# IST-DASLab/qutlass

Measured on AMD Instinct MI355X. Metric: TFLOP/s & %FP4-MFMA-peak, MXFP4 GEMM 4096x4096x4096, 1 MI355X, higher is better.
Workload: dtype fp4 (e2m1 x e2m1, e8m0 block scales, fp32 accumulate, bf16 out); 1 GPU; matmul_mxf4_bf16_tn 4096x4096x4096, gs=32 e8m0 scales (BASELINE.json configs[1]); parallelism=single GPU, clock_ramp=8000 untimed steps (~250 ms) before the 5 warmup steps

## Files before the change

qutlass_amd/csrc/capi.hip:

```cpp
#include <hip/hip_runtime.h>

#include <algorithm>
#include <atomic>
#include <chrono>
#include <cstdarg>
#include <cstdio>
#include <cstring>

#include "../../include/qutlass_amd.h"
#include "gemm_mx.hip.h"
#include "gemm_mx_deepp.hip.h"
#if QAMD_BENCH
#include "lab/gemm_mx_duo.hip.h"
#include "lab/gemm_mx_deepp_lab.hip.h"
#endif
#include "gemm_mx_skinny.hip.h"
#include "gemm_mx_ks.hip.h"
#include "gemm_mx_os.hip.h"
#include "gemm_mx_fusedq.hip.h"
#include "gemm_nvf4.hip.h"
#include "gemm_nvf4_pk.hip.h"
#include "gemm_nvf4_os.hip.h"
#include "quantize.hip.h"
#include "moe_route.hip.h"
#include "to_blocked.hip.h"
#include "transpose_u8.hip.h"
#include "quartet_bwd.hip.h"
#if QAMD_BENCH
#include "lab/quartet_bwd_lab.hip.h"
#endif

using namespace qamd;

#ifndef QAMD_TU
#define QAMD_TU 0
#endif
#define QAMD_DEF(n) (QAMD_TU == 0 || QAMD_TU == (n))
#ifndef QAMD_BENCH
#define QAMD_BENCH 0
#endif

namespace qamd_host {

#if QAMD_DEF(1)
thread_local char g_err[512] = "";
#if QAMD_BENCH
std::atomic<int> g_hw_fp4_cvt{1};
std::atomic<int> g_gemm_variant{0};
std::atomic<int> g_nvf4_variant{0};
std::atomic<int> g_splitk_wg{0};
std::atomic<int> g_splitk_min_kt{32};
std::atomic<int> g_transpose_nc{0};
std::atomic<int> g_pp_shift{2};
std::atomic<int> g_pp_flags{1};
std::atomic<int> g_quant_wg_per_cu{0};
std::atomic<int> g_deepp_grid{0};
std::atomic<int> g_bwd_variant{0};
std::atomic<int> g_moe_sort_one_launch_max{0};
std::atomic<int> g_splitk_force{0};
std::atomic<uint32_t*> g_dbg{nullptr};
#endif

int fail(int code, const char* fmt, ...) {
  va_list ap;
  va_start(ap, fmt);
  vsnprintf(g_err, sizeof(g_err), fmt, ap);
  va_end(ap);
  return code;
}

int check_launch(const char* what) {
  hipError_t e = hipGetLastError();
  if (e != hipSuccess) return fail(QAMD_ERR_HIP, "%s: %s", what, hipGetErrorString(e));
  return QAMD_OK;
}

unsigned long long next_launch_tag() {
  static std::atomic<unsigned long long> tag{[] {
    unsigned long long x = (unsigned long long)std::chrono::steady_clock::now().time_since_epoch().count() ^ ((unsigned long long)(uintptr_t)&g_err << 17);
    x ^= x >> 31; x *= 0x9e3779b97f4a7c15ull; x ^= x >> 29;
    return x | 1ull;
  }()};
  return tag.fetch_add(1, std::memory_order_relaxed) + 1;
}
#else
unsigned long long next_launch_tag();
#if QAMD_BENCH
extern std::atomic<int> g_hw_fp4_cvt, g_gemm_variant, g_nvf4_variant, g_splitk_wg, g_splitk_min_kt, g_transpose_nc, g_pp_shift, g_pp_flags, g_quant_wg_per_cu, g_splitk_force, g_deepp_grid, g_bwd_variant, g_moe_sort_one_launch_max;
extern std::atomic<uint32_t*> g_dbg;
#endif
int fail(int code, const char* fmt, ...);
int check_launch(const char* what);
#endif

#if QAMD_BENCH
inline bool opt_hw_fp4() { return g_hw_fp4_cvt.load() != 0; }
inline int opt_gemm_variant() { return g_gemm_variant.load(); }
inline int opt_nvf4_variant() { return g_nvf4_variant.load(); }
inline int opt_splitk_wg() { return g_splitk_wg.load(); }
inline int opt_splitk_min_kt() { return g_splitk_min_kt.load(); }
inline int opt_transpose_nc() { return g_transpose_nc.load(); }
inline int opt_pp_shift() { return g_pp_shift.load(); }
inline int opt_pp_flags() { return g_pp_flags.load(); }
inline int opt_quant_wg_per_cu() { return g_quant_wg_per_cu.load(); }
inline int opt_splitk_force() { return g_splitk_force.load(); }
inline int opt_deepp_grid() { return g_deepp_grid.load(); }
inline int opt_bwd_variant() { return g_bwd_variant.load(); }
inline int opt_moe_sort_one_launch_max() { return g_moe_sort_one_launch_max.load(); }
inline uint32_t* opt_dbg() { return g_dbg.load(); }
#else
constexpr bool opt_hw_fp4() { return true; }
constexpr int opt_gemm_variant() { return 0; }
constexpr int opt_nvf4_variant() { return 0; }
constexpr int opt_splitk_wg() { return 0; }
constexpr int opt_splitk_min_kt() { return 32; }
constexpr int opt_transpose_nc() { return 0; }
constexpr int opt_pp_shift() { return 2; }
constexpr int opt_pp_flags() { return 1; }
constexpr int opt_quant_wg_per_cu() { return 0; }
constexpr int opt_splitk_force() { return 0; }
constexpr int opt_deepp_grid() { return 0; }
constexpr int opt_bwd_variant() { return 0; }
constexpr int opt_moe_sort_one_launch_max() { return 0; }
constexpr uint32_t* opt_dbg() { return nullptr; }
#endif

inline int64_t cdiv(int64_t a, int64_t b) { return (a + b - 1) / b; }

#if QAMD_DEF(1)
int chip_cus() {
  static std::atomic<int> cache[64];
  int dev = 0;
  if (hipGetDevice(&dev) != hipSuccess || dev < 0 || dev >= 64) return 256;
  int v = cache[dev].load(std::memory_order_relaxed);
  if (v <= 0) {
    int n = 0;
    if (hipDeviceGetAttribute(&n, hipDeviceAttributeMultiprocessorCount, dev) != hipSuccess || n <= 0) n = 256;
// ... 834 lines not shown
  if (M * N >= (1ll << 40) || M >= (1ll << 31) || N >= (1ll << 31)) return fail(QAMD_ERR_INVALID, "%s: an output of 2^40 elements is not supported", name);
  return QAMD_OK;
}

template <int EBITS>
int gemm_mx(const char* name, const void* A, const void* B, const void* A_sf, const void* B_sf,
            const float* alpha, void* D, int64_t M, int64_t N, int64_t K, void* stream, void* ws = nullptr, int64_t ws_bytes = 0, int a_fmt = 0) {
  if (int rc = mx_check(name, EBITS, A, B, A_sf, B_sf, alpha, D, M, N, K)) return rc;
  const MxArgs x{A, B, A_sf, B_sf, alpha, D, K, N, EBITS, false};
  return for_each_range(name, M, N, K * EBITS / 8, 256, [&](int64_t r0, int64_t c0, int64_t m, int64_t n) -> int {
    const MxPlan pl = mx_plan<EBITS>(a_fmt, m, n, K, N, ws ? ws_bytes : 0, chip_cus());
    for (int i = 0; i < pl.n; ++i)
      if (int rc = mx_launch<EBITS>(name, pl.l[i], mx_params(x, r0, c0 + pl.l[i].c0, m, pl.l[i].n), ws, a_fmt, (hipStream_t)stream)) return rc;
    return QAMD_OK;
  });
}

template <class P>
int debug_plan(const char* name, int64_t M, int64_t N, int64_t rowbytes, int gran, int* out, int cap, P&& plan) {
  int cnt = 0;
  const int rc = for_each_range(name, M, N, rowbytes, gran, [&](int64_t, int64_t, int64_t m, int64_t n) {
    const MxPlan pl = plan(m, n);
    for (int i = 0; i < pl.n; ++i, ++cnt)
      if (cnt < 8 && cnt < cap) { out[3 * cnt] = pl.l[i].variant; out[3 * cnt + 1] = (int)pl.l[i].n; out[3 * cnt + 2] = pl.l[i].splits; }
    return QAMD_OK;
  });
  return rc == QAMD_OK ? cnt : -1;
}

#endif

enum QuantKind { QK_PLAIN, QK_GATED, QK_GATHER, QK_GATED_GSCALE, QK_GATHER_GSCALE };

template <int KIND, int R, bool NV, int METHOD, bool MASK, bool BLK>
int launch_quant(const QuantParams& p, hipStream_t s, int grid) {
  static_assert((KIND != QK_GATED_GSCALE && KIND != QK_GATHER_GSCALE) || (NV && METHOD == METHOD_ABSMAX && !MASK && !BLK), "per-expert global scales: NV abs-max, flat scales");
  if constexpr (KIND == QK_GATED_GSCALE) {
    hipLaunchKernelGGL((fused_silu_mul_quantize_gscale_kernel<R>), dim3(grid), dim3(256), 0, s, p);
    return check_launch("fused_silu_mul_quantize_gscale_kernel");
  } else if constexpr (KIND == QK_GATHER_GSCALE) {
    hipLaunchKernelGGL((fused_gather_quantize_gscale_kernel<R>), dim3(grid), dim3(256), 0, s, p);
    return check_launch("fused_gather_quantize_gscale_kernel");
  } else if constexpr (KIND == QK_GATED) {
    hipLaunchKernelGGL((fused_silu_mul_quantize_kernel<R, NV, METHOD, BLK>), dim3(grid), dim3(256), 0, s, p);
    return check_launch("fused_silu_mul_quantize_kernel");
  } else if constexpr (KIND == QK_GATHER) {
    hipLaunchKernelGGL((fused_gather_quantize_kernel<R, NV, METHOD>), dim3(grid), dim3(256), 0, s, p);
    return check_launch("fused_gather_quantize_kernel");
  } else {
#if QAMD_BENCH
    if (!opt_hw_fp4()) hipLaunchKernelGGL((fused_quantize_kernel<R, NV, METHOD, MASK, false, BLK>), dim3(grid), dim3(256), 0, s, p);
    else
#endif
    hipLaunchKernelGGL((fused_quantize_kernel<R, NV, METHOD, MASK, true, BLK>), dim3(grid), dim3(256), 0, s, p);
    return check_launch("fused_quantize_kernel");
  }
}

template <int KIND, bool NV, int METHOD, bool MASK, bool BLK>
int dispatch_quant(int rot, const QuantParams& p, hipStream_t s, int grid, const char* name) {
  static_assert(!MASK || (KIND == QK_PLAIN && !NV && METHOD == METHOD_QUEST), "the clip mask exists for the plain MX quest quantizer only");
  static_assert(!BLK || (KIND != QK_GATHER && KIND != QK_GATED_GSCALE && KIND != QK_GATHER_GSCALE), "the gathering and the grouped-scale quantizers write flat scales only");
  switch (rot) {
    case 16:
      if constexpr (NV) return launch_quant<KIND, 16, NV, METHOD, false, BLK>(p, s, grid);
      break;
    case 32: return launch_quant<KIND, 32, NV, METHOD, MASK, BLK>(p, s, grid);
    case 64:
      if constexpr (!MASK) return launch_quant<KIND, 64, NV, METHOD, false, BLK>(p, s, grid);
// ... 46 lines not shown
  if (which == 4) {
    if (!hw) { QAMD_BWD_GO((bwd_qt_panel_kernel<false>), 512); return check_launch("bwd_qt_panel_kernel"); }
    QAMD_BWD_GO((bwd_qt_panel_kernel<true>), 512);
    return check_launch("bwd_qt_panel_kernel");
  }
#endif
  if (which == 1) {
#if QAMD_BENCH
    if (!hw) { if (qt) QAMD_BWD_GO((bwd_quant_t_kernel<true, false>), 512); else QAMD_BWD_GO((bwd_quant_t_kernel<false, false>), 512); return check_launch("bwd_quant_t_kernel"); }
#endif
    if (qt) QAMD_BWD_GO((bwd_quant_t_kernel<true, true>), 512); else QAMD_BWD_GO((bwd_quant_t_kernel<false, true>), 512);
    return check_launch("bwd_quant_t_kernel");
  }
#if QAMD_BENCH
  if (!hw) {
    if (which == 3) { if (qt) QAMD_BWD_GO((bwd_quant_tw_kernel<true, false, 8>), 256); else QAMD_BWD_GO((bwd_quant_tw_kernel<false, false, 8>), 256); }
    else            { if (qt) QAMD_BWD_GO((bwd_quant_tw_kernel<true, false, 4>), 256); else QAMD_BWD_GO((bwd_quant_tw_kernel<false, false, 4>), 256); }
    return check_launch("bwd_quant_tw_kernel");
  }
  if (which == 9) {
    if (qt) QAMD_BWD_GO((bwd_quant_tw_kernel<true, true, 2>), 256); else QAMD_BWD_GO((bwd_quant_tw_kernel<false, true, 2>), 256);
    return check_launch("bwd_quant_tw_kernel");
  }
  if (qt && which == 3) { QAMD_BWD_GO((bwd_quant_tw_kernel<true, true, 8>), 256); return check_launch("bwd_quant_tw_kernel"); }
  if (!qt && which == 2) { QAMD_BWD_GO((bwd_quant_tw_kernel<false, true, 4>), 256); return check_launch("bwd_quant_tw_kernel"); }
#endif
  if (qt) QAMD_BWD_GO((bwd_quant_tw_kernel<true, true, 4>), 256); else QAMD_BWD_GO((bwd_quant_tw_kernel<false, true, 8>), 256);
#undef QAMD_BWD_GO
  return check_launch("bwd_quant_tw_kernel");
}
#endif

#if QAMD_DEF(1)
int quant_grid(int ntiles, int rot) {
  int per_cu = opt_quant_wg_per_cu();
  if (per_cu <= 0) per_cu = rot >= 128 ? 2 : (rot >= 64 ? 4 : 8);
  int g = (ntiles + 3) / 4;
  const int cap = chip_cus() * per_cu;
  return g < 1 ? 1 : (g > cap ? cap : g);
}

int blocked_pad_grid(int grid, int sf_rows, int sf_cols) {
  const int64_t prow = cdiv(sf_rows, 128) * 128, cb = cdiv(sf_cols, 4);
  const int64_t stores = (prow - sf_rows) * cb + (int64_t)sf_rows * (cb * 4 - sf_cols);
  const int64_t want = std::min<int64_t>(cdiv(stores, 256), chip_cus());
  return (int)std::max<int64_t>(grid, want);
}

inline int quant_check_rot(const char* name, const QuantFormat& f, int rot, bool mask = false) {
  if (f.has_rot(rot)) return QAMD_OK;
  return fail(QAMD_ERR_INVALID, "%s: Unsupported rotation size %d; expected %s.", name, rot, mask ? "32" : f.rots);
}

inline int quant_check_method(const char* name, int method) {
  if (method == QAMD_METHOD_QUEST || method == QAMD_METHOD_ABSMAX) return QAMD_OK;
  return fail(QAMD_ERR_INVALID, "%s: invalid method %d", name, method);
}

inline int quant_check_h(const char* name, int rot, const void* h) {
  if (rot < 64 || (uintptr_t)h % 16 == 0) return QAMD_OK;
  return fail(QAMD_ERR_INVALID, "%s: the rotation matrix must be 16-byte aligned for rotation sizes >= 64", name);
}

inline int quant_rp(int rot) { return rot < 32 ? 32 : rot; }

inline int quant_fill(QuantParams& p, const QuantFormat& f, int rot, int64_t numel, int64_t k, bool blocked, const int32_t* src_row = nullptr, int64_t src_n = 0) {
  p.numel = numel;
  p.ntiles = (int)cdiv(numel, (int64_t)quant_rp(rot) * 32);
  p.sf_rows = blocked ? (int)(numel / k) : 0; p.sf_cols = blocked ? (int)(k / f.group) : 0;
  p.src_row = src_row; p.src_n = (int)src_n;
  const int grid = quant_grid(p.ntiles, rot);
  return blocked ? blocked_pad_grid(grid, p.sf_rows, p.sf_cols) : grid;
}

struct QuantGroups {
  const int32_t* offs;
  int64_t e;
};
static_assert(qamd::QUANT_MAX_E == qamd::GRP_MAX_E, "the quantizers take as many experts as the grouped GEMMs");

inline int quant_check_groups(const char* name, const QuantGroups& g) {
  if (g.e < 1 || g.e > qamd::QUANT_MAX_E) return fail(QAMD_ERR_INVALID, "%s: E must be in [1, %d] (got %lld)", name, qamd::QUANT_MAX_E, (long long)g.e);
  if ((uintptr_t)g.offs % 4) return fail(QAMD_ERR_INVALID, "%s: offs must be 4-byte aligned", name);
  return QAMD_OK;
}

template <int KIND>
int select_quant(bool nv, int method, bool mask, bool blocked, int rot, const QuantParams& p, hipStream_t s, int grid, const char* name) {
  auto go = [&](auto nv_, auto method_, auto mask_) {
    using NV = decltype(nv_); using M = decltype(method_); using K = decltype(mask_);
    if constexpr (KIND != QK_GATHER)
      if (blocked) return dispatch_quant<KIND, NV::value, M::value, K::value, true>(rot, p, s, grid, name);
    return dispatch_quant<KIND, NV::value, M::value, K::value, false>(rot, p, s, grid, name);
  };
  using Quest = std::integral_constant<int, METHOD_QUEST>; using AbsMax = std::integral_constant<int, METHOD_ABSMAX>;
  if constexpr (KIND == QK_PLAIN)
    if (mask) return go(std::false_type{}, Quest{}, std::true_type{});
  if (nv) return method == QAMD_METHOD_QUEST ? go(std::true_type{}, Quest{}, std::false_type{}) : go(std::true_type{}, AbsMax{}, std::false_type{});
  return method == QAMD_METHOD_QUEST ? go(std::false_type{}, Quest{}, std::false_type{}) : go(std::false_type{}, AbsMax{}, std::false_type{});
}

template <int KIND>
int select_quant_grouped(int method, int rot, QuantParams& p, const QuantGroups& g, hipStream_t s, int grid, const char* name) {
  if (method == QAMD_METHOD_QUEST) return select_quant<KIND>(true, method, false, false, rot, p, s, grid, name);
// ... 319 lines not shown
static int gated_common_check(const char* name, const void* x, int64_t rows, int64_t inter, int64_t align) {
  if (rows < 0 || inter <= 0 || rows >= (1ll << 31) || inter >= (1ll << 31)) return fail(QAMD_ERR_INVALID, "%s: bad shape (%lld, 2 * %lld)", name, (long long)rows, (long long)inter);
  if (inter % align) return fail(QAMD_ERR_INVALID, "%s: the gate / up width %lld must be a multiple of %lld", name, (long long)inter, (long long)align);
  if ((uintptr_t)x % 16) return fail(QAMD_ERR_INVALID, "%s: x must be 16-byte aligned", name);
  return QAMD_OK;
}

int qutlass_amd_silu_mul_bf16(const void* x, int64_t rows, int64_t inter, void* out, void* stream) {
  const char* name = "silu_and_mul";
  if (int rc = gated_common_check(name, x, rows, inter, 8)) return rc;
  if ((uintptr_t)out % 16) return fail(QAMD_ERR_INVALID, "%s: out must be 16-byte aligned", name);
  if (rows == 0) return QAMD_OK;
  if (!x || !out) return fail(QAMD_ERR_INVALID, "%s: null pointer argument", name);
  SiluMulParams p;
  p.x = (const uint16_t*)x; p.out = (uint16_t*)out; p.chunks = rows * (inter / 8); p.cpr = (uint32_t)(inter / 8);
  const int grid = (int)std::min<int64_t>(cdiv(p.chunks, 256), (int64_t)chip_cus() * 8);
  hipLaunchKernelGGL(silu_mul_bf16_kernel<0>, dim3(grid), dim3(256), 0, (hipStream_t)stream, p);
  return check_launch("silu_mul_bf16_kernel");
}

static int fused_silu_mul_quantize_impl(const char* name, const QuantFormat& f, const void* x, const void* h, int rot, int64_t rows, int64_t inter, int method,
                                        const float* global_scale, int blocked, void* out_e2m1, void* out_sf, void* stream, const QuantGroups* grp = nullptr) {
  if (int rc = quant_check_rot(name, f, rot)) return rc;
  if (int rc = quant_check_method(name, method)) return rc;
  if (int rc = gated_common_check(name, x, rows, inter, quant_rp(rot))) return rc;
  if (rows * inter >= (1ll << 29)) return fail(QAMD_ERR_INVALID, "%s: x (rows * 2 * inter * 2 = %lld bytes) must stay below 2 GiB", name, (long long)(rows * inter * 4));
  if (rows == 0) return QAMD_OK;
  if (!x || !h || !out_e2m1 || !out_sf || (f.nv && !global_scale) || (grp && !grp->offs)) return fail(QAMD_ERR_INVALID, "%s: null pointer argument", name);
  if (int rc = quant_check_h(name, rot, h)) return rc;
  if (grp) if (int rc = quant_check_groups(name, *grp)) return rc;
  QuantParams p;
  p.x = (const uint16_t*)x; p.h = (const uint16_t*)h; p.out = (uint8_t*)out_e2m1; p.out_sf = (uint8_t*)out_sf;
  p.out_mask = nullptr; p.global_scale = global_scale; p.inter = (int)inter;
  const int grid = quant_fill(p, f, rot, rows * inter, inter, blocked != 0);
  if (grp) return select_quant_grouped<QK_GATED>(method, rot, p, *grp, (hipStream_t)stream, grid, name);
  return select_quant<QK_GATED>(f.nv, method, false, blocked != 0, rot, p, (hipStream_t)stream, grid, name);
}

int qutlass_amd_fused_silu_mul_quantize_mx(const void* x, const void* h, int rot, int64_t rows, int64_t inter, int method, int blocked, void* out_e2m1,
                                           void* out_e8m0, void* stream) {
  return fused_silu_mul_quantize_impl(blocked ? "fusedSiluMulQuantizeMxBlocked" : "fusedSiluMulQuantizeMx", kQuantMx, x, h, rot, rows, inter, method, nullptr, blocked,
                                      out_e2m1, out_e8m0, stream);
}

int qutlass_amd_fused_silu_mul_quantize_nv(const void* x, const void* h, int rot, int64_t rows, int64_t inter, int method, const float* global_scale, int blocked,
                                           void* out_e2m1, void* out_e4m3, void* stream) {
  return fused_silu_mul_quantize_impl(blocked ? "fusedSiluMulQuantizeNvBlocked" : "fusedSiluMulQuantizeNv", kQuantNv, x, h, rot, rows, inter, method, global_scale,
                                      blocked, out_e2m1, out_e4m3, stream);
}

static int fused_gather_quantize_impl(const char* name, const QuantFormat& f, const void* x, const void* h, int rot, int64_t t, int64_t k, const int32_t* src_row,
                                      int64_t m, int method, const float* global_scale, void* out_e2m1, void* out_sf, void* stream, const QuantGroups* grp = nullptr) {
  if (int rc = quant_check_rot(name, f, rot)) return rc;
  if (int rc = quant_check_method(name, method)) return rc;
  if (t < 0 || m < 0 || k <= 0 || t >= (1ll << 31) || m >= (1ll << 31) || k >= (1ll << 31))
    return fail(QAMD_ERR_INVALID, "%s: bad shape (x (%lld, %lld), %lld indices)", name, (long long)t, (long long)k, (long long)m);
  if (k % quant_rp(rot)) return fail(QAMD_ERR_INVALID, "%s: the row length %lld must be a multiple of %d", name, (long long)k, quant_rp(rot));
  if ((uintptr_t)x % 16 || (uintptr_t)src_row % 4) return fail(QAMD_ERR_INVALID, "%s: x must be 16-byte aligned (and src_row 4-byte aligned)", name);
  if (t * k >= (1ll << 30)) return fail(QAMD_ERR_INVALID, "%s: x (rows * k * 2 = %lld bytes) must stay below 2 GiB", name, (long long)(t * k * 2));
  if (m * k >= (1ll << 31)) return fail(QAMD_ERR_INVALID, "%s: more than 2^31 elements is not supported", name);
  if (m == 0) return QAMD_OK;
  if ((!x && t > 0) || !h || !src_row || !out_e2m1 || !out_sf || (f.nv && !global_scale) || (grp && !grp->offs)) return fail(QAMD_ERR_INVALID, "%s: null pointer argument", name);
  if (int rc = quant_check_h(name, rot, h)) return rc;
  if (grp) if (int rc = quant_check_groups(name, *grp)) return rc;
  QuantParams p;
  p.x = (const uint16_t*)x; p.h = (const uint16_t*)h; p.out = (uint8_t*)out_e2m1; p.out_sf = (uint8_t*)out_sf;
  p.out_mask = nullptr; p.global_scale = global_scale; p.inter = (int)k;
// ... 514 lines not shown
    if (u.mode < 0) break;
    if (n < cap) { out[5 * n] = u.tile; out[5 * n + 1] = u.kb; out[5 * n + 2] = u.ke; out[5 * n + 3] = u.mode; out[5 * n + 4] = u.slot; }
    ++n;
  }
  return n;
}
int qutlass_amd_debug_nvf4_pk_units(int w, int grid, int T, int sk_tiles, int KT, int* out, int cap) { return qutlass_amd_debug_sk_units(w, grid, T, sk_tiles, KT, 1, out, cap); }

#if QAMD_BENCH
void qutlass_amd_debug_set_trace_buffer(void* p) { g_dbg.store((uint32_t*)p); }
#endif

const char* qutlass_amd_last_error(void) { return g_err; }
#if QAMD_BENCH
const char* qutlass_amd_version(void) { return "qutlass_amd 0.2.0 (gfx950, lab build)"; }
#else
const char* qutlass_amd_version(void) { return "qutlass_amd 0.2.0 (gfx950)"; }
#endif

int qutlass_amd_set_option(const char* key, int value) {
  if (!key) return -1;
  (void)value;
#if QAMD_BENCH
  if (!strcmp(key, "hw_fp4_cvt")) return g_hw_fp4_cvt.exchange(value);
  if (!strcmp(key, "gemm_variant")) return g_gemm_variant.exchange(value);
  if (!strcmp(key, "nvf4_variant")) return g_nvf4_variant.exchange(value);
  if (!strcmp(key, "transpose_nc")) return g_transpose_nc.exchange(value);
  if (!strcmp(key, "splitk_wg")) return g_splitk_wg.exchange(value);
  if (!strcmp(key, "splitk_min_kt")) return g_splitk_min_kt.exchange(value);
  if (!strcmp(key, "splitk_force")) return g_splitk_force.exchange(value);
  if (!strcmp(key, "deepp_grid")) return g_deepp_grid.exchange(value);
  if (!strcmp(key, "bwd_variant")) return g_bwd_variant.exchange(value);
  if (!strcmp(key, "quant_wg_per_cu")) return g_quant_wg_per_cu.exchange(value);
  if (!strcmp(key, "moe_sort_one_launch_max")) return g_moe_sort_one_launch_max.exchange(value);
  if (!strcmp(key, "pp_shift")) return g_pp_shift.exchange(value);
  if (!strcmp(key, "pp_flags")) return g_pp_flags.exchange(value);
#endif
  return -1;
}

}
#pragma GCC visibility pop
#endif
```

qutlass_amd/csrc/quantize.hip.h:

```cpp
#pragma once
#include "common.hip.h"

namespace qamd {

enum { METHOD_QUEST = 0, METHOD_ABSMAX = 1 };

struct QuantParams {
  const uint16_t* x;
  const uint16_t* h;
  uint8_t* out;
  uint8_t* out_sf;
  uint32_t* out_mask;
  const float* global_scale;
  int64_t numel;
  int ntiles;
  int sf_rows, sf_cols;
  int inter = 0;
  const int32_t* src_row = nullptr;
  int src_n = 0;
  int E = 0;
  const int32_t* offs = nullptr;
};

__host__ __device__ __forceinline__ int quant_group_of_row(const int32_t* offs, int E, int m) {
// ... 160 lines not shown
__device__ __forceinline__ v4i silu_mul8(const v4i g, const v4i u) {
  uint32_t sw[4], need = 0;
#pragma unroll
  for (int i = 0; i < 4; ++i) {
    const uint32_t gw = (uint32_t)g[i];
    const float g0 = __uint_as_float(gw << 16), g1 = __uint_as_float(gw & 0xffff0000u);
    const float s0 = silu_f32(g0), s1 = silu_f32(g1);
    sw[i] = pack_bf16x2(s0, s1);
    need |= (silu_needs_fp64(g0, s0) ? 1u : 0u) << (2 * i) | (silu_needs_fp64(g1, s1) ? 1u : 0u) << (2 * i + 1);
  }
  if (__builtin_expect(need != 0, 0)) {
#pragma nounroll
    for (int i = 0; i < 8; ++i) {
      if (need & (1u << i)) {
        const int w = i >> 1;
        const uint32_t gw = (uint32_t)(w == 0 ? g[0] : w == 1 ? g[1] : w == 2 ? g[2] : g[3]);
        const double gd = (double)__uint_as_float((i & 1) ? (gw & 0xffff0000u) : (gw << 16));
        const uint32_t r = f64_to_bf16_bits(gd / (1.0 + exp(-gd)));
        const uint32_t keep = (i & 1) ? 0x0000ffffu : 0xffff0000u, val = (i & 1) ? (r << 16) : r;
#pragma unroll
        for (int k = 0; k < 4; ++k) sw[k] = (k == w) ? ((sw[k] & keep) | val) : sw[k];
      }
    }
  }
  v4i r;
#pragma unroll
  for (int i = 0; i < 4; ++i) {
    const uint32_t uw = (uint32_t)u[i];
    r[i] = (int)pack_bf16x2(__uint_as_float(sw[i] << 16) * __uint_as_float(uw << 16), __uint_as_float(sw[i] & 0xffff0000u) * __uint_as_float(uw & 0xffff0000u));
  }
  return r;
}

template <int R, bool NV, int METHOD, bool MASK, bool HWCVT, bool BLK = false, bool PAD = true, bool GATED = false, bool GATHER = false, bool GSCALE = false>
__device__ __forceinline__ void fused_quantize_body(const QuantParams& p, const int bid, const int nblk) {
  constexpr int RP = (R < 32) ? 32 : R;
  constexpr int KC = RP / 16;
  constexpr int JT = RP / 32;
  constexpr bool HTR = RP >= 64;
  constexpr int HROW = HTR ? RP * 2 + 64 : RP * 2 + 16;
  __shared__ __attribute__((aligned(16))) char hT[RP * HROW];
  constexpr bool STAGED = RP >= 64;
  constexpr int XROW = RP * 2 + 16;
  __shared__ __attribute__((aligned(16))) char xs_all[STAGED ? 4 * 32 * XROW : 16];

  const int tid = threadIdx.x, lane = tid & 63, wave = uniform(tid >> 6);
  const int row = lane & 31, half = lane >> 5;

  const int64_t ngroups = p.numel / (NV ? 16 : 32);
  static_assert(!(GATED && GATHER) && !(GATHER && (BLK || MASK)), "the gathering form: plain operand, flat scales, no clip mask");
  static_assert(!GSCALE || (NV && METHOD == METHOD_ABSMAX && !BLK && !MASK && (GATED || GATHER)), "per-expert global scales: NV abs-max, flat scales, gathering or gated");
  const __amdgpu_buffer_rsrc_t rx = make_rsrc(p.x, GATHER ? (uint32_t)p.src_n * (uint32_t)p.inter * 2u : (uint32_t)(p.numel * (GATED ? 4 : 2)));

  const int wave_global = bid * 4 + wave, nwaves = nblk * 4;
  v4i xnext[RP / 16];
  v4i unext[GATED ? RP / 16 : 1];
  const int lane_off = STAGED ? lane * 16 : row * RP * 2 + half * 16;
  constexpr int LSTEP = STAGED ? 1024 : 32;
  char* xs = xs_all + (STAGED ? wave * 32 * XROW : 0);
  uint32_t g_row = 0, g_rem = 0, g_qstep = 0, g_rstep = 0, g_rpr = 1, g_nrows = 0;
  float g_rc = 1.0f;
  uint32_t s_row = 0, s_rem = 0, n_rem = 0;
  float gs_next = 1.0f;
  if constexpr (GATED || GATHER) {
    g_rpr = (uint32_t)p.inter / RP;
    g_rc = __builtin_amdgcn_rcpf((float)g_rpr);
    g_nrows = (uint32_t)(p.numel / RP);
    const uint32_t r0 = (uint32_t)wave_global * 32u, step = (uint32_t)nwaves * 32u;
    g_row = r0 / g_rpr;
    g_rem = r0 - g_row * g_rpr;
    g_qstep = step / g_rpr;
    g_rstep = step - g_qstep * g_rpr;
    if constexpr (GSCALE) { s_row = g_row; s_rem = g_rem; }
  }
  auto gated_off = [&](const int t, const uint32_t lrow, const uint32_t cb) -> int {
    const uint32_t x = g_rem + lrow;
    uint32_t q = (uint32_t)((float)x * g_rc);
    int32_t r = (int32_t)(x - q * g_rpr);
    if (r < 0) { q -= 1; r += (int32_t)g_rpr; }
    if (r >= (int32_t)g_rpr) { q += 1; r -= (int32_t)g_rpr; }
    const uint32_t off = (g_row + q) * ((uint32_t)p.inter * 4u) + (uint32_t)r * (RP * 2u) + cb;
    return ((uint32_t)t * 32u + lrow < g_nrows) ? (int)off : (int)0xfffffff0u;
  };
  auto gated_loads = [&](const int t) {
    if constexpr (STAGED) {
      constexpr int CPR = RP / 8;
#pragma unroll
      for (int i = 0; i < RP / 16; ++i) {
        const int q = i * 64 + lane;
        const int off = gated_off(t, (uint32_t)(q / CPR), (uint32_t)(q % CPR) * 16u);
        xnext[i] = __builtin_amdgcn_raw_buffer_load_b128(rx, off, 0, 0);
        unext[i] = __builtin_amdgcn_raw_buffer_load_b128(rx, off, p.inter * 2, 0);
      }
    } else {
      const int off = gated_off(t, (uint32_t)row, (uint32_t)half * 16u);
#pragma unroll
      for (int kc = 0; kc < RP / 16; ++kc) {
        xnext[kc] = __builtin_amdgcn_raw_buffer_load_b128(rx, off + kc * 32, 0, 0);
        unext[kc] = __builtin_amdgcn_raw_buffer_load_b128(rx, off + kc * 32, p.inter * 2, 0);
      }
    }
    g_rem += g_rstep;
    const uint32_t carry = g_rem >= g_rpr ? 1u : 0u;
    g_rem -= carry ? g_rpr : 0u;
    g_row += g_qstep + carry;
  };
  const __amdgpu_buffer_rsrc_t ri = make_rsrc(GATHER ? (const void*)p.src_row : (const void*)p.x, GATHER ? (uint32_t)(p.numel / p.inter) * 4u : 0u);
  int gidx = 0;
  auto gather_index_load = [&]() { gidx = __builtin_amdgcn_raw_buffer_load_b32(ri, (int)((g_row + (uint32_t)row) * 4u), 0, 0); };
  auto gather_off = [&](const int t, const uint32_t lrow, const uint32_t cb) -> int {
    const uint32_t x = g_rem + lrow;
    uint32_t q = (uint32_t)((float)x * g_rc);
    int32_t r = (int32_t)(x - q * g_rpr);
    if (r < 0) { q -= 1; r += (int32_t)g_rpr; }
    if (r >= (int32_t)g_rpr) { q += 1; r -= (int32_t)g_rpr; }
    const uint32_t idx = (uint32_t)__builtin_amdgcn_ds_bpermute((int)(q * 4u), gidx);
    const bool ok = idx < (uint32_t)p.src_n && (uint32_t)t * 32u + lrow < g_nrows;
    return ok ? (int)(idx * ((uint32_t)p.inter * 2u) + (uint32_t)r * (RP * 2u) + cb) : (int)0x80000000u;
  };
  auto gather_loads = [&](const int t) {
    if constexpr (STAGED) {
      constexpr int CPR = RP / 8;
#pragma unroll
      for (int i = 0; i < RP / 16; ++i) {
        const int q = i * 64 + lane;
        xnext[i] = __builtin_amdgcn_raw_buffer_load_b128(rx, gather_off(t, (uint32_t)(q / CPR), (uint32_t)(q % CPR) * 16u), 0, 0);
      }
    } else {
      const int off = gather_off(t, (uint32_t)row, (uint32_t)half * 16u);
#pragma unroll
      for (int kc = 0; kc < RP / 16; ++kc) xnext[kc] = __builtin_amdgcn_raw_buffer_load_b128(rx, off + kc * 32, 0, 0);
    }
    g_rem += g_rstep;
    const uint32_t carry = g_rem >= g_rpr ? 1u : 0u;
    g_rem -= carry ? g_rpr : 0u;
    g_row += g_qstep + carry;
    gather_index_load();
  };
  if constexpr (GATHER) {
    gather_index_load();
  } else if constexpr (GATED) {
    gated_loads(wave_global);
  } else {
    const int xoff0 = (wave_global < p.ntiles) ? (int)((int64_t)wave_global * 32 * RP * 2) + lane_off : 0x7f000000;
#pragma unroll
    for (int kc = 0; kc < RP / 16; ++kc) xnext[kc] = __builtin_amdgcn_raw_buffer_load_b128(rx, xoff0 + kc * LSTEP, 0, 0);
  }
  int32_t ov[GSCALE ? QUANT_MAX_E / 256 : 1];
  if constexpr (GSCALE) {
#pragma unroll
    for (int i = 0; i < QUANT_MAX_E / 256; ++i) {
      const int idx = i * 256 + tid;
      if (i * 256 < p.E) ov[i] = p.offs[idx < p.E ? idx : p.E - 1];
    }
  }
  const float gscale = (NV && !GSCALE) ? *p.global_scale : 1.0f;
  const uint32_t sfCB = BLK ? ((uint32_t)p.sf_cols + 3u) >> 2 : 0u;
  if (BLK && PAD) {
    const uint32_t prow = ((uint32_t)p.sf_rows + 127u) & ~127u, pcol = sfCB * 4u;
    const uint32_t n1 = (prow - (uint32_t)p.sf_rows) * pcol, cpad = pcol - (uint32_t)p.sf_cols, n2 = (uint32_t)p.sf_rows * cpad;
    const uint32_t nd = n1 >> 2;
    for (uint32_t i = (uint32_t)bid * 256u + tid; i < nd + n2; i += (uint32_t)nblk * 256u) {
      if (i < nd) {
        const uint32_t r = (uint32_t)p.sf_rows + i / sfCB, cb = i % sfCB;
        *(uint32_t*)(p.out_sf + blocked_sf_offset(r, 4u * cb, sfCB)) = 0u;
      } else {
        const uint32_t j = i - nd, r = j / cpad, c = (uint32_t)p.sf_cols + j % cpad;
        p.out_sf[blocked_sf_offset(r, c, sfCB)] = 0;
      }
    }
  }

  if (R < 32) {
    constexpr int NE = RP * RP / 256;
    uint16_t hv[NE];
#pragma unroll
    for (int i = 0; i < NE; ++i) {
      const int idx = i * 256 + tid, k = idx / RP, j = idx % RP;
      hv[i] = p.h[(k & 15) * R + (j & 15)];
// ... 6 lines not shown
    }
  } else {
    if constexpr (HTR) {
      constexpr int NCH = RP * RP / 8 / 256, CPRH = RP / 8;
      v4i hc[NCH];
#pragma unroll
      for (int i = 0; i < NCH; ++i) hc[i] = *(const v4i*)(p.h + (i * 256 + tid) * 8);
      if constexpr (GATHER) gather_loads(wave_global);
#pragma unroll
      for (int i = 0; i < NCH; ++i) {
        const int c = i * 256 + tid;
        *(v4i*)(hT + (c / CPRH) * HROW + (c % CPRH) * 16) = hc[i];
      }
    } else {
      constexpr int NE = RP * RP / 256;
      uint16_t hv[NE];
#pragma unroll
      for (int i = 0; i < NE; ++i) hv[i] = p.h[i * 256 + tid];
      if constexpr (GATHER) gather_loads(wave_global);
#pragma unroll
      for (int i = 0; i < NE; ++i) {
        const int idx = i * 256 + tid, k = idx / RP, j = idx % RP;
        *(uint16_t*)(hT + j * HROW + k * 2) = hv[i];
      }
    }
  }
  if constexpr (GSCALE) {
    int32_t* so = quant_offs_lds();
#pragma unroll
    for (int i = 0; i < QUANT_MAX_E / 256; ++i)
      if (i * 256 < p.E) so[i * 256 + tid] = ov[i];
  }
  __syncthreads();
  auto gscale_lookup = [&]() {
    if constexpr (GSCALE) {
      const int g = quant_group_of_row(quant_offs_lds(), p.E, (int)(s_row + (uint32_t)row));
      gs_next = p.global_scale[g < 0 ? 0 : (g < p.E ? g : p.E - 1)];
      n_rem = s_rem;
      s_rem += g_rstep;
      const uint32_t carry = s_rem >= g_rpr ? 1u : 0u;
      s_rem -= carry ? g_rpr : 0u;
      s_row += g_qstep + carry;
    }
  };
  gscale_lookup();

  constexpr uint32_t SF_GPR = NV ? 2 * JT : JT;
  uint32_t sf_row = 0, sf_rem = 0, sf_qstep = 0, sf_rstep = 0, sf_rpr = 1;
  if (BLK) {
    sf_rpr = (uint32_t)p.sf_cols / SF_GPR;
    const uint32_t r0 = (uint32_t)wave_global * 32u + (uint32_t)row, step = (uint32_t)nwaves * 32u;
    sf_row = r0 / sf_rpr;
    sf_rem = r0 - sf_row * sf_rpr;
    sf_qstep = step / sf_rpr;
    sf_rstep = step - sf_qstep * sf_rpr;
  }
  for (int tile = wave_global; tile < p.ntiles; tile += nwaves) {
    int hoist_guard = 0;
    if (RP >= 64) asm volatile("" : "+v"(hoist_guard));
    const int64_t r_abs = (int64_t)tile * 32 + row;
    const uint32_t sf_col0 = BLK ? sf_rem * SF_GPR : 0u;
    v8bf xf[KC];
    const float gs_cur = gs_next;
    const uint32_t c_rem = n_rem;
    if constexpr (GATED) {
#pragma unroll
      for (int i = 0; i < KC; ++i) xnext[i] = silu_mul8(xnext[i], unext[i]);
    }
    if (STAGED) {
      constexpr int CPR = RP / 8;
#pragma unroll
      for (int i = 0; i < KC; ++i) {
        const int q = i * 64 + lane;
        *(v4i*)(xs + (q / CPR) * XROW + (q % CPR) * 16) = xnext[i];
      }
      __builtin_amdgcn_s_waitcnt(0xc07f);
      __builtin_amdgcn_wave_barrier();
#pragma unroll
      for (int kc = 0; kc < KC; ++kc) xf[kc] = *(const v8bf*)(xs + row * XROW + (2 * kc + half) * 16);
    } else {
#pragma unroll
      for (int kc = 0; kc < KC; ++kc) xf[kc] = __builtin_bit_cast(v8bf, xnext[kc]);
    }
    if constexpr (GATHER) {
      gather_loads(tile + nwaves);
    } else if constexpr (GATED) {
      gated_loads(tile + nwaves);
    } else {
      const int64_t on = (int64_t)(tile + nwaves) * 32 * RP * 2 + lane_off;
      const int xoffn = (tile + nwaves < p.ntiles) ? (int)on : 0x7f000000;
#pragma unroll
      for (int kc = 0; kc < KC; ++kc) xnext[kc] = __builtin_amdgcn_raw_buffer_load_b128(rx, xoffn + kc * LSTEP, 0, 0);
    }
    gscale_lookup();
    float gs = gscale;
    if constexpr (GSCALE) {
      const uint32_t x = c_rem + (uint32_t)row;
      uint32_t q = (uint32_t)((float)x * g_rc);
      const int32_t r = (int32_t)(x - q * g_rpr);
      q += r < 0 ? 0xffffffffu : (r >= (int32_t)g_rpr ? 1u : 0u);
      gs = __uint_as_float((uint32_t)__builtin_amdgcn_ds_bpermute((int)(q * 4u), (int)__float_as_uint(gs_cur)));
    }
#pragma unroll
    for (int jt = 0; jt < JT; ++jt) {
      v16f acc;
#pragma unroll
      for (int r = 0; r < 16; ++r) acc[r] = 0.f;
#pragma unroll
      for (int kc = 0; kc < KC; ++kc) {
        v8bf hf;
        if constexpr (HTR) {
          typedef short v4s_ __attribute__((ext_vector_type(4)));
          typedef __attribute__((address_space(3))) v4s_* lds_v4s_t;
          const char* tp = hT + hoist_guard + (8 * half + ((lane & 15) >> 2) + 16 * kc) * HROW + (((lane & 31) >> 4) * 16 + (lane & 3) * 4) * 2 + jt * 64;
          const v4s_ lo = __builtin_amdgcn_ds_read_tr16_b64_v4i16((lds_v4s_t)tp);
          const v4s_ hi = __builtin_amdgcn_ds_read_tr16_b64_v4i16((lds_v4s_t)(tp + 4 * HROW));
          const v8u16 hv8 = {(uint16_t)lo[0], (uint16_t)lo[1], (uint16_t)lo[2], (uint16_t)lo[3], (uint16_t)hi[0], (uint16_t)hi[1], (uint16_t)hi[2], (uint16_t)hi[3]};
          hf = __builtin_bit_cast(v8bf, hv8);
        } else {
          hf = *(const v8bf*)(hT + hoist_guard + (jt * 32 + row) * HROW + (kc * 16 + half * 8) * 2);
        }
        if constexpr (R < 32) {
          const v16f z = {0.f, 0.f, 0.f, 0.f, 0.f, 0.f, 0.f, 0.f, 0.f, 0.f, 0.f, 0.f, 0.f, 0.f, 0.f, 0.f};
          const v16f part = __builtin_amdgcn_mfma_f32_32x32x16_bf16(hf, xf[kc], z, 0, 0, 0);
#pragma unroll
          for (int r = 0; r < 8; ++r) acc[8 * kc + r] = part[8 * kc + r];
        } else {
          acc = __builtin_amdgcn_mfma_f32_32x32x16_bf16(hf, xf[kc], acc, 0, 0, 0);
        }
      }
      const int64_t grp32 = r_abs * JT + jt;

      if (!NV) {
        float scale;
        bool nan_risk;
        if (METHOD == METHOD_ABSMAX) {
          float m = 0.f;
#pragma unroll
          for (int r = 0; r < 16; ++r) m = fmaxf(m, fabsf(acc[r]));
          m = xhalf_max(m);
          scale = m + 1e-8f;
          nan_risk = m == 0.f;
        } else {
          float s1 = 0.f, s2 = 0.f;
// ... 133 lines not shown
    if (BLK) {
      sf_rem += sf_rstep;
      const uint32_t carry = sf_rem >= sf_rpr ? 1u : 0u;
      sf_rem -= carry ? sf_rpr : 0u;
      sf_row += sf_qstep + carry;
    }
  }
}

template <int R, bool NV, int METHOD, bool MASK, bool HWCVT, bool BLK = false>
__global__ __launch_bounds__(256) void fused_quantize_kernel(const QuantParams p) {
  fused_quantize_body<R, NV, METHOD, MASK, HWCVT, BLK>(p, (int)blockIdx.x, (int)gridDim.x);
}

template <int R, bool NV, int METHOD, bool BLK>
__global__ __launch_bounds__(256) void fused_silu_mul_quantize_kernel(const QuantParams p) {
  fused_quantize_body<R, NV, METHOD, false, true, BLK, true, true>(p, (int)blockIdx.x, (int)gridDim.x);
}

template <int R, bool NV, int METHOD>
__global__ __launch_bounds__(256) void fused_gather_quantize_kernel(const QuantParams p) {
  fused_quantize_body<R, NV, METHOD, false, true, false, true, false, true>(p, (int)blockIdx.x, (int)gridDim.x);
}

template <int R>
__global__ __launch_bounds__(256) void fused_gather_quantize_gscale_kernel(const QuantParams p) {
  fused_quantize_body<R, true, METHOD_ABSMAX, false, true, false, true, false, true, true>(p, (int)blockIdx.x, (int)gridDim.x);
}
template <int R>
__global__ __launch_bounds__(256) void fused_silu_mul_quantize_gscale_kernel(const QuantParams p) {
  fused_quantize_body<R, true, METHOD_ABSMAX, false, true, false, true, true, false, true>(p, (int)blockIdx.x, (int)gridDim.x);
}

struct SiluMulParams {
  const uint16_t* x;
  uint16_t* out;
  int64_t chunks;
  uint32_t cpr;
};
template <int UNUSED = 0>
__global__ __launch_bounds__(256) void silu_mul_bf16_kernel(const SiluMulParams p) {
  const uint32_t first = blockIdx.x * 256u + threadIdx.x, step = gridDim.x * 256u;
  uint32_t row = first / p.cpr, cc = first - row * p.cpr;
  const uint32_t qstep = step / p.cpr, rstep = step - qstep * p.cpr;
  for (int64_t c = first; c < p.chunks; c += step) {
    const uint16_t* g = p.x + ((int64_t)row * 2 * p.cpr + cc) * 8;
    const v4i gv = *(const v4i*)g, uv = *(const v4i*)(g + (int64_t)p.cpr * 8);
    *(v4i*)(p.out + c * 8) = silu_mul8(gv, uv);
    cc += rstep;
    const uint32_t carry = cc >= p.cpr ? 1u : 0u;
    cc -= carry ? p.cpr : 0u;
    row += qstep + carry;
  }
}

struct MoeCombineParams {
  const uint16_t* y;
  const int32_t* pos;
  const float* w;
  uint16_t* out;
  int64_t chunks;
  uint32_t cpr;
  uint32_t m;
  int topk;
};
template <int UNUSED = 0>
// ... 47 lines not shown
```

Before: 4386 TFLOP/s.

## Split rotated quantize tiles across waves with register-resident Hadamard fragments

For rotation sizes of 64 and above, adds a split form of the fused quantize kernels. Several waves of a workgroup cooperate on one tile, each computing one 32-column slice of the rotation, and each wave preloads its Hadamard fragment into registers once instead of reading it from LDS on every tile. X staging moves to a shared double buffer synchronised with a block barrier. A heuristic, plus a new grid-sizing rule, picks the split form for gated inputs or small tile counts. This adds block-wide barriers per tile in exchange for more parallelism per tile and less LDS traffic.

```diff
diff --git a/qutlass_amd/csrc/capi.hip b/qutlass_amd/csrc/capi.hip
--- a/qutlass_amd/csrc/capi.hip
+++ b/qutlass_amd/csrc/capi.hip
@@ -54,6 +54,7 @@
 std::atomic<int> g_pp_shift{2};
 std::atomic<int> g_pp_flags{1};
 std::atomic<int> g_quant_wg_per_cu{0};
+std::atomic<int> g_quant_form{0};
 std::atomic<int> g_deepp_grid{0};
 std::atomic<int> g_bwd_variant{0};
 std::atomic<int> g_moe_sort_one_launch_max{0};
@@ -86,7 +87,7 @@
 #else
 unsigned long long next_launch_tag();
 #if QAMD_BENCH
-extern std::atomic<int> g_hw_fp4_cvt, g_gemm_variant, g_nvf4_variant, g_splitk_wg, g_splitk_min_kt, g_transpose_nc, g_pp_shift, g_pp_flags, g_quant_wg_per_cu, g_splitk_force, g_deepp_grid, g_bwd_variant, g_moe_sort_one_launch_max;
+extern std::atomic<int> g_hw_fp4_cvt, g_gemm_variant, g_nvf4_variant, g_splitk_wg, g_splitk_min_kt, g_transpose_nc, g_pp_shift, g_pp_flags, g_quant_wg_per_cu, g_quant_form, g_splitk_force, g_deepp_grid, g_bwd_variant, g_moe_sort_one_launch_max;
 extern std::atomic<uint32_t*> g_dbg;
 #endif
 int fail(int code, const char* fmt, ...);
@@ -103,6 +104,7 @@
 inline int opt_pp_shift() { return g_pp_shift.load(); }
 inline int opt_pp_flags() { return g_pp_flags.load(); }
 inline int opt_quant_wg_per_cu() { return g_quant_wg_per_cu.load(); }
+inline int opt_quant_form() { return g_quant_form.load(); }
 inline int opt_splitk_force() { return g_splitk_force.load(); }
 inline int opt_deepp_grid() { return g_deepp_grid.load(); }
 inline int opt_bwd_variant() { return g_bwd_variant.load(); }
@@ -1003,9 +1005,26 @@
 
 enum QuantKind { QK_PLAIN, QK_GATED, QK_GATHER, QK_GATED_GSCALE, QK_GATHER_GSCALE };
 
+inline bool quant_split(bool gated, int ntiles, int rot, int cus) {
+#if QAMD_BENCH
+  if (opt_quant_form() > 0 && rot >= 64) return opt_quant_form() == 2;
+#endif
+  return rot >= 64 && (gated || ntiles <= 16 * cus);
+}
+
 template <int KIND, int R, bool NV, int METHOD, bool MASK, bool BLK>
 int launch_quant(const QuantParams& p, hipStream_t s, int grid) {
   static_assert((KIND != QK_GATED_GSCALE && KIND != QK_GATHER_GSCALE) || (NV && METHOD == METHOD_ABSMAX && !MASK && !BLK), "per-expert global scales: NV abs-max, flat scales");
+  if constexpr (R >= 64) {
+    if (quant_split(KIND == QK_GATED || KIND == QK_GATED_GSCALE, p.ntiles, R, chip_cus())) {
+      if constexpr (KIND == QK_GATED_GSCALE) hipLaunchKernelGGL((fused_silu_mul_quantize_gscale_split_kernel<R>), dim3(grid), dim3(256), 0, s, p);
+      else if constexpr (KIND == QK_GATHER_GSCALE) hipLaunchKernelGGL((fused_gather_quantize_gscale_split_kernel<R>), dim3(grid), dim3(256), 0, s, p);
+      else if constexpr (KIND == QK_GATED) hipLaunchKernelGGL((fused_silu_mul_quantize_split_kernel<R, NV, METHOD, BLK>), dim3(grid), dim3(256), 0, s, p);
+      else if constexpr (KIND == QK_GATHER) hipLaunchKernelGGL((fused_gather_quantize_split_kernel<R, NV, METHOD>), dim3(grid), dim3(256), 0, s, p);
+      else hipLaunchKernelGGL((fused_quantize_split_kernel<R, NV, METHOD, BLK>), dim3(grid), dim3(256), 0, s, p);
+      return check_launch("fused_quantize_split_kernel");
+    }
+  }
   if constexpr (KIND == QK_GATED_GSCALE) {
     hipLaunchKernelGGL((fused_silu_mul_quantize_gscale_kernel<R>), dim3(grid), dim3(256), 0, s, p);
     return check_launch("fused_silu_mul_quantize_gscale_kernel");
@@ -1118,8 +1137,16 @@
 #endif
 
 #if QAMD_DEF(1)
-int quant_grid(int ntiles, int rot) {
+int quant_grid(int ntiles, int rot, bool gated, bool gscale) {
   int per_cu = opt_quant_wg_per_cu();
+  if (quant_split(gated, ntiles, rot, chip_cus())) {
+    if (per_cu <= 0) per_cu = rot >= 128 ? (gated ? (gscale ? 3 : 4) : 2) : (gated ? 7 : 4);
+    const int tpw = rot >= 128 ? 1 : 2, cap = chip_cus() * per_cu;
+    const int g = (ntiles + tpw - 1) / tpw;
+    if (g <= cap) return g < 1 ? 1 : g;
+    const int trips = (g + cap - 1) / cap;
+    return (g + trips - 1) / trips;
+  }
   if (per_cu <= 0) per_cu = rot >= 128 ? 2 : (rot >= 64 ? 4 : 8);
   int g = (ntiles + 3) / 4;
   const int cap = chip_cus() * per_cu;
@@ -1150,12 +1177,13 @@
 
 inline int quant_rp(int rot) { return rot < 32 ? 32 : rot; }
 
-inline int quant_fill(QuantParams& p, const QuantFormat& f, int rot, int64_t numel, int64_t k, bool blocked, const int32_t* src_row = nullptr, int64_t src_n = 0) {
+inline int quant_fill(QuantParams& p, const QuantFormat& f, int rot, int64_t numel, int64_t k, bool blocked, const int32_t* src_row = nullptr, int64_t src_n = 0,
+                      bool gated = false, bool gscale = false) {
   p.numel = numel;
   p.ntiles = (int)cdiv(numel, (int64_t)quant_rp(rot) * 32);
   p.sf_rows = blocked ? (int)(numel / k) : 0; p.sf_cols = blocked ? (int)(k / f.group) : 0;
   p.src_row = src_row; p.src_n = (int)src_n;
-  const int grid = quant_grid(p.ntiles, rot);
+  const int grid = quant_grid(p.ntiles, rot, gated, gscale);
   return blocked ? blocked_pad_grid(grid, p.sf_rows, p.sf_cols) : grid;
 }
 
@@ -1541,7 +1569,7 @@
   QuantParams p;
   p.x = (const uint16_t*)x; p.h = (const uint16_t*)h; p.out = (uint8_t*)out_e2m1; p.out_sf = (uint8_t*)out_sf;
   p.out_mask = nullptr; p.global_scale = global_scale; p.inter = (int)inter;
-  const int grid = quant_fill(p, f, rot, rows * inter, inter, blocked != 0);
+  const int grid = quant_fill(p, f, rot, rows * inter, inter, blocked != 0, nullptr, 0, true, grp && method == QAMD_METHOD_ABSMAX);
   if (grp) return select_quant_grouped<QK_GATED>(method, rot, p, *grp, (hipStream_t)stream, grid, name);
   return select_quant<QK_GATED>(f.nv, method, false, blocked != 0, rot, p, (hipStream_t)stream, grid, name);
 }
@@ -2122,6 +2150,7 @@
   if (!strcmp(key, "deepp_grid")) return g_deepp_grid.exchange(value);
   if (!strcmp(key, "bwd_variant")) return g_bwd_variant.exchange(value);
   if (!strcmp(key, "quant_wg_per_cu")) return g_quant_wg_per_cu.exchange(value);
+  if (!strcmp(key, "quant_form")) return g_quant_form.exchange(value);
   if (!strcmp(key, "moe_sort_one_launch_max")) return g_moe_sort_one_launch_max.exchange(value);
   if (!strcmp(key, "pp_shift")) return g_pp_shift.exchange(value);
   if (!strcmp(key, "pp_flags")) return g_pp_flags.exchange(value);
diff --git a/qutlass_amd/csrc/quantize.hip.h b/qutlass_amd/csrc/quantize.hip.h
--- a/qutlass_amd/csrc/quantize.hip.h
+++ b/qutlass_amd/csrc/quantize.hip.h
@@ -216,17 +216,23 @@
   return r;
 }
 
-template <int R, bool NV, int METHOD, bool MASK, bool HWCVT, bool BLK = false, bool PAD = true, bool GATED = false, bool GATHER = false, bool GSCALE = false>
+template <int R, bool NV, int METHOD, bool MASK, bool HWCVT, bool BLK = false, bool PAD = true, bool GATED = false, bool GATHER = false, bool GSCALE = false, bool WSPLIT = false>
 __device__ __forceinline__ void fused_quantize_body(const QuantParams& p, const int bid, const int nblk) {
   constexpr int RP = (R < 32) ? 32 : R;
   constexpr int KC = RP / 16;
   constexpr int JT = RP / 32;
   constexpr bool HTR = RP >= 64;
   constexpr int HROW = HTR ? RP * 2 + 64 : RP * 2 + 16;
-  __shared__ __attribute__((aligned(16))) char hT[RP * HROW];
+  constexpr bool SPLIT = RP >= 64 && WSPLIT;
+  static_assert(RP >= 64 || !WSPLIT, "the split form exists for R >= 64");
+  constexpr int WPT = SPLIT ? JT : 1;
+  constexpr int TPW = 4 / WPT;
+  constexpr int NX = KC / WPT;
+  constexpr int XROW = RP * 2 + 16;
+  constexpr int HBYTES = RP * HROW, XSPLIT = TPW * 2 * 32 * XROW;
+  __shared__ __attribute__((aligned(16))) char hT[SPLIT && XSPLIT > HBYTES ? XSPLIT : HBYTES];
   constexpr bool STAGED = RP >= 64;
-  constexpr int XROW = RP * 2 + 16;
-  __shared__ __attribute__((aligned(16))) char xs_all[STAGED ? 4 * 32 * XROW : 16];
+  __shared__ __attribute__((aligned(16))) char xs_all[STAGED && !SPLIT ? 4 * 32 * XROW : 16];
 
   const int tid = threadIdx.x, lane = tid & 63, wave = uniform(tid >> 6);
   const int row = lane & 31, half = lane >> 5;
@@ -236,12 +242,13 @@
   static_assert(!GSCALE || (NV && METHOD == METHOD_ABSMAX && !BLK && !MASK && (GATED || GATHER)), "per-expert global scales: NV abs-max, flat scales, gathering or gated");
   const __amdgpu_buffer_rsrc_t rx = make_rsrc(p.x, GATHER ? (uint32_t)p.src_n * (uint32_t)p.inter * 2u : (uint32_t)(p.numel * (GATED ? 4 : 2)));
 
-  const int wave_global = bid * 4 + wave, nwaves = nblk * 4;
-  v4i xnext[RP / 16];
-  v4i unext[GATED ? RP / 16 : 1];
-  const int lane_off = STAGED ? lane * 16 : row * RP * 2 + half * 16;
-  constexpr int LSTEP = STAGED ? 1024 : 32;
-  char* xs = xs_all + (STAGED ? wave * 32 * XROW : 0);
+  const int ws = SPLIT ? wave % WPT : 0;
+  const int wave_global = SPLIT ? bid * TPW + wave / WPT : bid * 4 + wave, nwaves = SPLIT ? nblk * TPW : nblk * 4;
+  v4i xnext[NX];
+  v4i unext[GATED ? NX : 1];
+  const int lane_off = STAGED ? (ws * 64 + lane) * 16 : row * RP * 2 + half * 16;
+  constexpr int LSTEP = STAGED ? 1024 * WPT : 32;
+  char* xs = SPLIT ? hT + (wave / WPT) * (2 * 32 * XROW) : xs_all + (STAGED ? wave * 32 * XROW : 0);
   uint32_t g_row = 0, g_rem = 0, g_qstep = 0, g_rstep = 0, g_rpr = 1, g_nrows = 0;
   float g_rc = 1.0f;
   uint32_t s_row = 0, s_rem = 0, n_rem = 0;
@@ -270,8 +277,8 @@
     if constexpr (STAGED) {
       constexpr int CPR = RP / 8;
 #pragma unroll
-      for (int i = 0; i < RP / 16; ++i) {
-        const int q = i * 64 + lane;
+      for (int i = 0; i < NX; ++i) {
+        const int q = (i * WPT + ws) * 64 + lane;
         const int off = gated_off(t, (uint32_t)(q / CPR), (uint32_t)(q % CPR) * 16u);
         xnext[i] = __builtin_amdgcn_raw_buffer_load_b128(rx, off, 0, 0);
         unext[i] = __builtin_amdgcn_raw_buffer_load_b128(rx, off, p.inter * 2, 0);
@@ -306,8 +313,8 @@
     if constexpr (STAGED) {
       constexpr int CPR = RP / 8;
 #pragma unroll
-      for (int i = 0; i < RP / 16; ++i) {
-        const int q = i * 64 + lane;
+      for (int i = 0; i < NX; ++i) {
+        const int q = (i * WPT + ws) * 64 + lane;
         xnext[i] = __builtin_amdgcn_raw_buffer_load_b128(rx, gather_off(t, (uint32_t)(q / CPR), (uint32_t)(q % CPR) * 16u), 0, 0);
       }
     } else {
@@ -328,7 +335,7 @@
   } else {
     const int xoff0 = (wave_global < p.ntiles) ? (int)((int64_t)wave_global * 32 * RP * 2) + lane_off : 0x7f000000;
 #pragma unroll
-    for (int kc = 0; kc < RP / 16; ++kc) xnext[kc] = __builtin_amdgcn_raw_buffer_load_b128(rx, xoff0 + kc * LSTEP, 0, 0);
+    for (int kc = 0; kc < NX; ++kc) xnext[kc] = __builtin_amdgcn_raw_buffer_load_b128(rx, xoff0 + kc * LSTEP, 0, 0);
   }
   int32_t ov[GSCALE ? QUANT_MAX_E / 256 : 1];
   if constexpr (GSCALE) {
@@ -401,6 +408,20 @@
       if (i * 256 < p.E) so[i * 256 + tid] = ov[i];
   }
   __syncthreads();
+  v8bf hreg[SPLIT ? KC : 1];
+  if constexpr (SPLIT) {
+    typedef short v4s_ __attribute__((ext_vector_type(4)));
+    typedef __attribute__((address_space(3))) v4s_* lds_v4s_t;
+#pragma unroll
+    for (int kc = 0; kc < KC; ++kc) {
+      const char* tp = hT + (8 * half + ((lane & 15) >> 2) + 16 * kc) * HROW + (((lane & 31) >> 4) * 16 + (lane & 3) * 4) * 2 + ws * 64;
+      const v4s_ lo = __builtin_amdgcn_ds_read_tr16_b64_v4i16((lds_v4s_t)tp);
+      const v4s_ hi = __builtin_amdgcn_ds_read_tr16_b64_v4i16((lds_v4s_t)(tp + 4 * HROW));
+      const v8u16 hv8 = {(uint16_t)lo[0], (uint16_t)lo[1], (uint16_t)lo[2], (uint16_t)lo[3], (uint16_t)hi[0], (uint16_t)hi[1], (uint16_t)hi[2], (uint16_t)hi[3]};
+      hreg[kc] = __builtin_bit_cast(v8bf, hv8);
+    }
+    __syncthreads();
+  }
   auto gscale_lookup = [&]() {
     if constexpr (GSCALE) {
       const int g = quant_group_of_row(quant_offs_lds(), p.E, (int)(s_row + (uint32_t)row));
@@ -424,9 +445,10 @@
     sf_qstep = step / sf_rpr;
     sf_rstep = step - sf_qstep * sf_rpr;
   }
-  for (int tile = wave_global; tile < p.ntiles; tile += nwaves) {
+  int xstep = 32 * XROW;
+  for (int tile = wave_global; (SPLIT ? tile - wave / WPT : tile) < p.ntiles; tile += nwaves) {
     int hoist_guard = 0;
-    if (RP >= 64) asm volatile("" : "+v"(hoist_guard));
+    if (RP >= 64 && !SPLIT) asm volatile("" : "+v"(hoist_guard));
     const int64_t r_abs = (int64_t)tile * 32 + row;
     const uint32_t sf_col0 = BLK ? sf_rem * SF_GPR : 0u;
     v8bf xf[KC];
@@ -434,19 +456,24 @@
     const uint32_t c_rem = n_rem;
     if constexpr (GATED) {
 #pragma unroll
-      for (int i = 0; i < KC; ++i) xnext[i] = silu_mul8(xnext[i], unext[i]);
+      for (int i = 0; i < NX; ++i) xnext[i] = silu_mul8(xnext[i], unext[i]);
     }
     if (STAGED) {
       constexpr int CPR = RP / 8;
 #pragma unroll
-      for (int i = 0; i < KC; ++i) {
-        const int q = i * 64 + lane;
+      for (int i = 0; i < NX; ++i) {
+        const int q = (i * WPT + ws) * 64 + lane;
         *(v4i*)(xs + (q / CPR) * XROW + (q % CPR) * 16) = xnext[i];
       }
-      __builtin_amdgcn_s_waitcnt(0xc07f);
-      __builtin_amdgcn_wave_barrier();
+      if constexpr (SPLIT) {
+        asm volatile("s_waitcnt lgkmcnt(0)\n\ts_barrier" ::: "memory");
+      } else {
+        __builtin_amdgcn_s_waitcnt(0xc07f);
+        __builtin_amdgcn_wave_barrier();
+      }
 #pragma unroll
       for (int kc = 0; kc < KC; ++kc) xf[kc] = *(const v8bf*)(xs + row * XROW + (2 * kc + half) * 16);
+      if constexpr (SPLIT) { xs += xstep; xstep = -xstep; }
     } else {
 #pragma unroll
       for (int kc = 0; kc < KC; ++kc) xf[kc] = __builtin_bit_cast(v8bf, xnext[kc]);
@@ -459,7 +486,7 @@
       const int64_t on = (int64_t)(tile + nwaves) * 32 * RP * 2 + lane_off;
       const int xoffn = (tile + nwaves < p.ntiles) ? (int)on : 0x7f000000;
 #pragma unroll
-      for (int kc = 0; kc < KC; ++kc) xnext[kc] = __builtin_amdgcn_raw_buffer_load_b128(rx, xoffn + kc * LSTEP, 0, 0);
+      for (int kc = 0; kc < NX; ++kc) xnext[kc] = __builtin_amdgcn_raw_buffer_load_b128(rx, xoffn + kc * LSTEP, 0, 0);
     }
     gscale_lookup();
     float gs = gscale;
@@ -471,14 +498,17 @@
       gs = __uint_as_float((uint32_t)__builtin_amdgcn_ds_bpermute((int)(q * 4u), (int)__float_as_uint(gs_cur)));
     }
 #pragma unroll
-    for (int jt = 0; jt < JT; ++jt) {
+    for (int jj = 0; jj < JT / WPT; ++jj) {
+      const int jt = SPLIT ? ws : jj;
       v16f acc;
 #pragma unroll
       for (int r = 0; r < 16; ++r) acc[r] = 0.f;
 #pragma unroll
       for (int kc = 0; kc < KC; ++kc) {
         v8bf hf;
-        if constexpr (HTR) {
+        if constexpr (SPLIT) {
+          hf = hreg[kc];
+        } else if constexpr (HTR) {
           typedef short v4s_ __attribute__((ext_vector_type(4)));
           typedef __attribute__((address_space(3))) v4s_* lds_v4s_t;
           const char* tp = hT + hoist_guard + (8 * half + ((lane & 15) >> 2) + 16 * kc) * HROW + (((lane & 31) >> 4) * 16 + (lane & 3) * 4) * 2 + jt * 64;
@@ -678,6 +708,27 @@
   fused_quantize_body<R, true, METHOD_ABSMAX, false, true, false, true, true, false, true>(p, (int)blockIdx.x, (int)gridDim.x);
 }
 
+template <int R, bool NV, int METHOD, bool BLK>
+__global__ __launch_bounds__(256) void fused_quantize_split_kernel(const QuantParams p) {
+  fused_quantize_body<R, NV, METHOD, false, true, BLK, true, false, false, false, true>(p, (int)blockIdx.x, (int)gridDim.x);
+}
+template <int R, bool NV, int METHOD, bool BLK>
+__global__ __launch_bounds__(256) void fused_silu_mul_quantize_split_kernel(const QuantParams p) {
+  fused_quantize_body<R, NV, METHOD, false, true, BLK, true, true, false, false, true>(p, (int)blockIdx.x, (int)gridDim.x);
+}
+template <int R, bool NV, int METHOD>
+__global__ __launch_bounds__(256) void fused_gather_quantize_split_kernel(const QuantParams p) {
+  fused_quantize_body<R, NV, METHOD, false, true, false, true, false, true, false, true>(p, (int)blockIdx.x, (int)gridDim.x);
+}
+template <int R>
+__global__ __launch_bounds__(256) void fused_gather_quantize_gscale_split_kernel(const QuantParams p) {
+  fused_quantize_body<R, true, METHOD_ABSMAX, false, true, false, true, false, true, true, true>(p, (int)blockIdx.x, (int)gridDim.x);
+}
+template <int R>
+__global__ __launch_bounds__(256) void fused_silu_mul_quantize_gscale_split_kernel(const QuantParams p) {
+  fused_quantize_body<R, true, METHOD_ABSMAX, false, true, false, true, true, false, true, true>(p, (int)blockIdx.x, (int)gridDim.x);
+}
+
 struct SiluMulParams {
   const uint16_t* x;
   uint16_t* out;
```

Result: no change. 4373 TFLOP/s (-0.3%).
